# data-mermaid/mermaid-classifier

Hardware: AMD Instinct MI355X
Metric: patches/sec (224x224 EfficientNet-B0) (higher is better)
Workload: dtype f16; 1 GPU; EfficientNet-B0 forward, batch=256 random 224x224 u8 patches per GPU -> (256,1280) fp32; per_gpu_batch=256, global_batch=256, weights=synthetic seed 0, input_batches_rotated=8, lanes_per_gpu=2, parallelism=patch-sharded x1

## Files before the change

### mermaid_classifier_amd/csrc/k_mid.hip

```cpp
#include "device_common.h"

template <int CKS, int KSD, int CE>
__global__ __launch_bounds__(512) void mid14_kernel(Mid14Args a)
{
    constexpr int HW = 196, CH = 96, NCHK = CE / CH, NPF = 13, NTILE = 6 * NPF, NBAND = 5;
    constexpr int ES2 = 416;
    constexpr int R = KSD / 2, NP = KSD == 5 ? 3 : 2;
    static_assert(CE % CH == 0, "chunking");
    extern __shared__ __attribute__((aligned(16))) unsigned char smem[];
    constexpr int ZT = R, ZB = R + 1;
    unsigned char* E = smem + ZT * 7 * ES2;
    float* pband = reinterpret_cast<float*>(smem + (98 + 7 * (ZT + ZB)) * ES2);
    const int tid = threadIdx.x, lane = tid & 63, wave = __builtin_amdgcn_readfirstlane(tid >> 6);
    const int m = lane & 15, q = lane >> 4;
    const int b = blockIdx.x;
    const int Cin = a.Cin;
    const GLOBAL_AS _Float16* wexp = sgpr_ptr<_Float16>(a.wexp);
    const GLOBAL_AS float* bexp = sgpr_ptr<float>(a.bexp);
    const GLOBAL_AS uint32_t* dwp = sgpr_ptr<uint32_t>(a.dwp);
    const GLOBAL_AS float* bdw = sgpr_ptr<float>(a.bdw);
    const int npf = wave < 5 ? 2 : 1;
    const int pf0 = wave < 5 ? 2 * wave : wave + 5;
    const GLOBAL_AS _Float16* xgp = sgpr_ptr<_Float16>(a.X) + (size_t)b * HW * Cin;
    const int band0 = tid / CH, cd = tid - band0 * CH;
// ... 119 lines not shown
                        } else {
                            wq[0][0] = r0 << 16; wq[0][1] = __builtin_amdgcn_alignbit(r1, r0, 16); wq[0][2] = 0u;
                            wq[1][0] = r0; wq[1][1] = r1; wq[1][2] = 0u;
                        }
#pragma unroll
                        for (int ip = 0; ip < NP; ++ip)
#pragma unroll
                            for (int ox = 0; ox < 14; ++ox) {
                                const int fp = (KSD == 5 || !(ox & 1)) ? (ox >> 1) - 1 : (ox >> 1);
                                const int xpc = fp + ip;
                                if (xpc < 0 || xpc > 6) continue;
                                if (!started[ox]) { acc[ox] = dot2_from(P[ro + ky][xpc], wq[ox & 1][ip], dbias); started[ox] = true; }
                                else acc[ox] = __builtin_amdgcn_fdot2(*reinterpret_cast<const h2*>(&P[ro + ky][xpc]),
                                                                      *reinterpret_cast<const h2*>(&wq[ox & 1][ip]), acc[ox], false);
                            }
                    }
                    silu_scaled_staged(acc);
#pragma unroll
                    for (int ox = 0; ox < 14; ox += 2) {
                        const f2 v = {acc[ox], acc[ox + 1]};
                        psum2 = psum2 + v;
                        const uint32_t hv = cvt_pk_f16(acc[ox], acc[ox + 1]);
                        dg[(size_t)(oy * 14 + ox) * CE] = (uint16_t)hv;
                        dg[(size_t)(oy * 14 + ox + 1) * CE] = (uint16_t)(hv >> 16);
                    }
                }
            }
            pband[band * CH + cd] = (psum2.x + psum2.y) + 0.f;
        }
        T7_BAR();
        if (tid < CH)
            a.pool[(size_t)b * CE + chunk * CH + tid] =
                ((pband[tid] + pband[CH + tid]) + pband[2 * CH + tid]) + pband[3 * CH + tid] + pband[4 * CH + tid];
    }
}

template <int CKS, int KSD, int CE, bool CHAIN>
static __device__ __forceinline__ void mid14m_body(const Mid14Args& args, const int chain_tid)
{
    const Mid14Args a = args;
    constexpr bool DBG = !CHAIN;
    const int tid = CHAIN ? chain_tid : (int)threadIdx.x;
    const int by = CHAIN ? 0 : (int)blockIdx.y, ny = CHAIN ? 1 : (int)gridDim.y;
    constexpr int HW = 196, NG = CE / 16, R = KSD / 2;
    constexpr int XSTR = 64 * CKS + 16;
    constexpr int ERS = 40;
    constexpr int ECS = 736;
    constexpr int EREG = 16 * ECS;
    constexpr int TREG = 56 * 32;
    extern __shared__ __attribute__((aligned(16))) unsigned char smem[];
    unsigned char* XS = smem;
    const int lane = tid & 63, wave = __builtin_amdgcn_readfirstlane(tid >> 6);
    unsigned char* EW = smem + HW * XSTR + wave * (EREG + TREG);
    unsigned char* TW = EW + EREG;
    const int n16 = lane & 15, q = lane >> 4;
    const int blk = lane >> 2, n = lane & 3;
    const int c = 2 * (blk & 3) + ((blk >> 2) & 1) + 8 * (blk >> 3);
    const int b = blockIdx.x;
    const int Cin = a.Cin;
    const GLOBAL_AS _Float16* wexp = sgpr_ptr<_Float16>(a.wexp);
    const GLOBAL_AS float* bexp = sgpr_ptr<float>(a.bexp);
    const GLOBAL_AS _Float16* dwt = sgpr_ptr<_Float16>(a.dwdiag);
    const GLOBAL_AS float* bdw = sgpr_ptr<float>(a.bdw);
    const bool clk = DBG && a.dbg_clk != nullptr;
    long long ck[5] = {clk ? (long long)__builtin_readcyclecounter() : 0, 0, 0, 0, 0};
    {
// ... 345 lines not shown
        dbg_clk[(size_t)b * 8 + 4] = (float)((long long)__builtin_readcyclecounter() - tk0);
        dbg_clk[(size_t)b * 8 + 5] = dbg_clk[(size_t)b * 8 + 4];
    }
    static_assert(NPAIR >= 7, "waves 0..6 all own a pair of pixel fragments");
    load_chunk(wave, 0, xc);
    PIN_VMEM();
    if (k2 < KP) {
        float a0 = be0, a1 = be1;
        f4 rq[7];
#pragma unroll
        for (int j = 0; j < 7; ++j) rq[j] = *reinterpret_cast<const f4*>(rs + 4 * j);
        __builtin_amdgcn_sched_barrier(0);
#pragma unroll
        for (int j = 0; j < 28; ++j) {
            const float r = j < CSP ? rq[j >> 2][j & 3] : 0.f;
            a0 = fma_mix_lo(w2[j], r, a0);
            a1 = fma_mix_hi(w2[j], r, a1);
        }
        {
            const float g0 = fc2_thr ? sigmoid_f(a0) : 0.f, g1 = fc2_thr ? sigmoid_f(a1) : 0.f;
            gate[k2] = g0;
            gate[k2 + 1] = g1;
            if (dbg_gate && fc2_thr) {
                dbg_gate[(size_t)b * K + k2] = g0;
                dbg_gate[(size_t)b * K + k2 + 1] = g1;
            }
        }
    }
    if (dbg_clk && tid == 0) dbg_clk[(size_t)b * 8 + 6] = (float)((long long)__builtin_readcyclecounter() - tk0);
    T7_BAR();
    }
    if (dbg_clk && tid == 0) dbg_clk[(size_t)b * 8 + 7] = (float)((long long)__builtin_readcyclecounter() - tk0);
    if (dbg_clk) tk1 = (long long)__builtin_readcyclecounter();
#pragma unroll 1
    for (int pr = wave; pr < NPAIR; pr += 8) {
        f4 acc[2][NF];
#pragma unroll
        for (int i = 0; i < 2; ++i)
#pragma unroll
            for (int nf = 0; nf < NF; ++nf) acc[i][nf] = bv[nf];
        h4 rv[2][NF];
        auto load_res = [&]() {
            if (!RES) return;
            const GLOBAL_AS _Float16* rg = sgpr_ptr<_Float16>(a.res) + (size_t)b * HW * a.N;
#pragma unroll
            for (int i = 0; i < 2; ++i) {
                const int p = 32 * pr + 16 * i + m;
                const int pc = p < HW ? p : HW - 1;
#pragma unroll
                for (int nf = 0; nf < NF; ++nf) {
                    const int c = 16 * nf + 4 * q;
                    rv[i][nf] = gload<h4>(rg, (unsigned)((pc * a.N + (c < a.N ? c : 0)) * 2));
                }
            }
        };
        if (EARLY_RES) load_res();
        h8 wcur[NF];
#pragma unroll
        for (int nf = 0; nf < NF; ++nf) wcur[nf] = *reinterpret_cast<const h8*>(wl + ((nf * KS) * 64 + lane) * 16);
        f4 gc0 = *reinterpret_cast<const f4*>(gate + 8 * q), gc1 = *reinterpret_cast<const f4*>(gate + 8 * q + 4);
        long long tka = 0;
        if (dbg_clk) tka = (long long)__builtin_readcyclecounter();
#pragma unroll
        for (int ch = 0; ch < NCH; ++ch) {
            if (ch + 1 < NCH) load_chunk(pr, ch + 1, xn);
            else load_chunk(pr + 8 < NPAIR ? pr + 8 : pr, 0, xn);
#pragma unroll
            for (int u = 0; u < CK; ++u) {
                const int ks = ch * CK + u;
                const int kn = ks + 1 < KS ? ks + 1 : 0;
                h8 wnx[NF];
#pragma unroll
                for (int nf = 0; nf < NF; ++nf) wnx[nf] = *reinterpret_cast<const h8*>(wl + ((nf * KS + kn) * 64 + lane) * 16);
                const f4 gn0 = *reinterpret_cast<const f4*>(gate + 32 * kn + 8 * q);
                const f4 gn1 = *reinterpret_cast<const f4*>(gate + 32 * kn + 8 * q + 4);
                PIN_VMEM();
                h8 xb[2];
#pragma unroll
                for (int i = 0; i < 2; ++i) {
                    const uint4 o = gate_h8(*reinterpret_cast<const uint4*>(&xc[i][u]), gc0, gc1);
                    xb[i] = *reinterpret_cast<const h8*>(&o);
                }
#pragma unroll
                for (int nf = 0; nf < NF; ++nf) {
                    acc[0][nf] = __builtin_amdgcn_mfma_f32_16x16x32_f16(wcur[nf], xb[0], acc[0][nf], 0, 0, 0);
                    acc[1][nf] = __builtin_amdgcn_mfma_f32_16x16x32_f16(wcur[nf], xb[1], acc[1][nf], 0, 0, 0);
                }
                PIN_VMEM();
#pragma unroll
                for (int nf = 0; nf < NF; ++nf) wcur[nf] = wnx[nf];
                gc0 = gn0;
                gc1 = gn1;
            }
#pragma unroll
            for (int i = 0; i < 2; ++i)
#pragma unroll
                for (int u = 0; u < CK; ++u) xc[i][u] = xn[i][u];
        }
        if (dbg_clk && tid == 0) dbg_clk[(size_t)b * 8 + 2] = (float)((long long)__builtin_readcyclecounter() - tka);
        if (!EARLY_RES) load_res();
#pragma unroll
        for (int i = 0; i < 2; ++i) {
            const int p = 32 * pr + 16 * i + m;
            if (p >= HW) continue;
#pragma unroll
            for (int nf = 0; nf < NF; ++nf) {
                const int c = 16 * nf + 4 * q;
                if (c >= a.N) continue;
                float v[4];
#pragma unroll
                for (int j = 0; j < 4; ++j) v[j] = acc[i][nf][j];
                if (RES) {
#pragma unroll
                    for (int j = 0; j < 4; ++j) v[j] += (float)rv[i][nf][j];
                }
                h4 o;
#pragma unroll
                for (int j = 0; j < 4; ++j) o[j] = (_Float16)v[j];
                *reinterpret_cast<h4*>(a.Y + ((size_t)b * HW + p) * a.N + c) = o;
            }
        }
    }
    if (dbg_clk) {
        T7_BAR();
        tk2 = (long long)__builtin_readcyclecounter();
        if (tid == 0) { dbg_clk[(size_t)b * 8] = (float)(tk1 - tk0); dbg_clk[(size_t)b * 8 + 1] = (float)(tk2 - tk1); }
    }
}

template <int KS, int NF, int HW, bool RES>
__global__ __launch_bounds__(512) void proj_patch_kernel(ProjPatchArgs a)
{
    proj_patch_body<KS, NF, HW, RES, false>(a, 0);
}

enum { CH_PP_15_5_R = 0, CH_MID_3_480 = 1, CH_PP_15_7 = 2, CH_MID_4_672 = 3, CH_PP_21_7_R = 4 };
__global__ __launch_bounds__(512) void chain14_kernel(Chain14Args c)
{
#pragma unroll 1
    for (int p = 0; p < c.nph; ++p) {
        const Chain14Phase& ph = c.ph[p];
        int tid = threadIdx.x;
        asm volatile("" : "+v"(tid));
        __builtin_assume(tid >= 0 && tid < 512);
        switch (ph.kind) {
        case CH_PP_15_5_R: proj_patch_body<15, 5, 196, true, true>(ph.pp, tid); break;
        case CH_MID_3_480: mid14m_body<3, 5, 480, true>(ph.mid, tid); break;
        case CH_PP_15_7: proj_patch_body<15, 7, 196, false, true>(ph.pp, tid); break;
        case CH_MID_4_672: mid14m_body<4, 5, 672, true>(ph.mid, tid); break;
        default: proj_patch_body<21, 7, 196, true, true>(ph.pp, tid); break;
        }
        __builtin_amdgcn_sched_barrier(0);
        __syncthreads();
// ... 22 lines not shown
#define PP(KS, NF, HW, RES) {{KS, NF, HW, RES}, "proj_patch<" #KS "," #NF "," #HW "," #RES ">", launch_proj_patch_t<KS, NF, HW, RES != 0>},
static const Inst<4, ProjPatchArgs> PROJ_PATCH_TABLE[] = {
    PP(5, 3, 784, 0)
    PP(8, 3, 784, 1)
    PP(8, 5, 196, 0)
    PP(15, 5, 196, 1)
    PP(15, 7, 196, 0)
    PP(21, 7, 196, 1)
    PP(6, 4, 784, 0)
    PP(12, 4, 784, 1)
    PP(12, 7, 196, 0)
};
#undef PP

const char* proj_patch_label(int K, int N, int HW, int res) { return inst_label(PROJ_PATCH_TABLE, {proj_patch_ksteps(K), (N + 15) / 16, HW, res}); }

int launch_proj_patch(const ProjPatchArgs& a, hipStream_t st)
{
    if (a.B < 1 || a.CSP < 4 || a.CSP > 28 || (a.CSP & 3) || a.nparts < 1) return -11;
    return inst_launch(PROJ_PATCH_TABLE, {proj_patch_ksteps(a.K), (a.N + 15) / 16, a.HW, a.res ? 1 : 0}, a, st, -5);
}

template <int CKS, int KSD, int CE>
static int launch_mid14_t(const Mid14Args& a, hipStream_t st)
{
    constexpr int ZROWS = 2 * (KSD / 2) + 1;
    const int lds = (98 + 7 * ZROWS) * 416 + 5 * 96 * 4 + 512;
    if (int r = set_max_lds<&mid14_kernel<CKS, KSD, CE>>(lds)) return r;
    hipLaunchKernelGGL((mid14_kernel<CKS, KSD, CE>), dim3(a.B, a.nsplit < 1 ? 1 : a.nsplit), dim3(512), lds, st, a);
    LAUNCH_CHECK();
    return 0;
}

template <int CKS, int KSD, int CE>
static int launch_mid14m_t(const Mid14Args& a, hipStream_t st)
{
    const int lds = 196 * (64 * CKS + 16) + 8 * (16 * 736 + 56 * 32);
    if (int r = set_max_lds<&mid14m_kernel<CKS, KSD, CE>>(lds)) return r;
    hipLaunchKernelGGL((mid14m_kernel<CKS, KSD, CE>), dim3(a.B, a.nsplit < 1 ? 1 : a.nsplit), dim3(512), lds, st, a);
    LAUNCH_CHECK();
    return 0;
}

#define MID14(CKS, KSD, CE) {{CKS, KSD, CE, 0}, "mid14<" #CKS "," #KSD "," #CE ",1>", launch_mid14_t<CKS, KSD, CE>},
#define MID14M(CKS, KSD, CE) {{CKS, KSD, CE, 1}, "mid14m<" #CKS "," #KSD "," #CE ",1>", launch_mid14m_t<CKS, KSD, CE>},
static const Inst<4, Mid14Args> MID14_TABLE[] = {
    MID14(4, 5, 672) MID14M(4, 5, 672)
    MID14(3, 5, 480) MID14M(3, 5, 480)
    MID14(3, 3, 480)
};
#undef MID14M
#undef MID14

const char* mid14_label(int Cin, int ks, int Ce, int dwm) { return inst_label(MID14_TABLE, {(Cin + 31) / 32, ks, Ce, dwm}); }

int launch_mid14(const Mid14Args& a, hipStream_t st)
{
    if (a.B < 1) return -14;
    return inst_launch(MID14_TABLE, {(a.Cin + 31) / 32, a.ks, a.Ce, a.dwdiag ? 1 : 0}, a, st, -5);
}

static int proj_patch_lds(int KS, int NF) { return NF * KS * 1024 + 2 * 32 * KS * 4 + 128; }
static int mid14m_lds(int CKS) { return 196 * (64 * CKS + 16) + 8 * (16 * 736 + 56 * 32); }

int chain14_proj_kind(int K, int N, int HW, int res)
{
    const int ks = proj_patch_ksteps(K), nf = (N + 15) / 16;
    if (HW != 196) return -1;
    if (ks == 15 && nf == 5 && res) return CH_PP_15_5_R;
    if (ks == 15 && nf == 7 && !res) return CH_PP_15_7;
    if (ks == 21 && nf == 7 && res) return CH_PP_21_7_R;
    return -1;
}

int chain14_mid_kind(int Cin, int ks, int Ce)
{
    const int cks = (Cin + 31) / 32;
    if (ks != 5) return -1;
    if (cks == 3 && Ce == 480) return CH_MID_3_480;
    if (cks == 4 && Ce == 672) return CH_MID_4_672;
    return -1;
}

int launch_chain14(const Chain14Args& a, hipStream_t st)
{
    if (a.B < 1 || a.nph < 1 || a.nph > CHAIN14_MAX_PHASES) return -14;
    int lds = 0;
    for (int p = 0; p < a.nph; ++p) {
        const Chain14Phase& ph = a.ph[p];
        int need;
        if (ph.kind == CH_MID_3_480 || ph.kind == CH_MID_4_672) {
            const Mid14Args& m = ph.mid;
// ... 16 lines not shown
```

### mermaid_classifier_amd/csrc/kernels.h

```cpp
#pragma once
#include <hip/hip_runtime.h>
#include <stdint.h>

#define LAUNCH_CHECK()                          \
    do {                                        \
        hipError_t e__ = hipGetLastError();     \
        if (e__ != hipSuccess) return (int)e__; \
    } while (0)

enum { EPI_SILU = 0, EPI_LINEAR = 1, EPI_GAP = 2 };


int mmc_fail(int code, const char* fmt, ...);

struct GemmArgs {
    const _Float16* X;
    int M, K;
    const _Float16* Wp;
    int Kp;
    const float* bias;
    _Float16* Y;
    int N;
    int mt, nt, n_chunks, defer_gate;
    int epi;
// ... 104 lines not shown
    int planar;
    float* pool;
    int B;
};
int launch_mb1(const Mb1Args& a, hipStream_t st);

struct MbtArgs {
    const _Float16* X;
    const _Float16* wexp;
    const float* bexp;
    const uint32_t* dwp;
    const float* bdw;
    _Float16* D;
    float* pool;
    int B, H, Cin, Ce, ks;
    int stride;
    const _Float16* dwtoe;
};
int launch_mbt(const MbtArgs& a, hipStream_t st);
const char* mbt_label(int H, int ks, int stride, int Cin, int Ce, int dw4);

struct Mid14Args {
    const _Float16* X;
    const _Float16* wexp;
    const float* bexp;
    const uint32_t* dwp;
    const float* bdw;
    _Float16* D;
    float* pool;
    int B, Cin, Ce, ks;
    int nsplit;
    float* dbg_clk;
    const _Float16* dwdiag;
};
int launch_mid14(const Mid14Args& a, hipStream_t st);
const char* mid14_label(int Cin, int ks, int Ce, int dwm);

struct ProjPatchArgs {
    const _Float16* X;
    const float* pool_part;
    const _Float16* wr_g;
    const float* br;
    const _Float16* we_t;
    const float* be;
    const _Float16* wfrag;
    const float* bias;
    const _Float16* res;
    _Float16* Y;
    float* dbg_gate;
    float* dbg_clk;
    int B, HW, K, N, CSP, nparts;
    float psc;
};
int launch_proj_patch(const ProjPatchArgs& a, hipStream_t st);
int proj_patch_ksteps(int K);
int proj_patch_fc1_rows(int K);
const char* proj_patch_label(int K, int N, int HW, int res);

enum { CHAIN14_MAX_PHASES = 7 };
struct Chain14Phase {
    int kind;
    union {
        ProjPatchArgs pp;
        Mid14Args mid;
    };
};
struct Chain14Args {
    int B, nph;
    Chain14Phase ph[CHAIN14_MAX_PHASES];
};
int chain14_proj_kind(int K, int N, int HW, int res);
int chain14_mid_kind(int Cin, int ks, int Ce);
int launch_chain14(const Chain14Args& a, hipStream_t st);

int launch_mbconv_a(const MbArgs& a, hipStream_t st);
const char* mbconv_a_label(const MbArgs& a);
const char* mbconv_pre_label(const MbArgs& a);
const char* mbconv_d_label(const MbArgs& a);
int launch_mbconv_pre(const MbArgs& a, const _Float16* pre_w, const float* pre_b, const float* pre_gate, hipStream_t st);
int launch_mbconv_d(const MbArgs& a, hipStream_t st);
int launch_stem(const uint8_t* patches, const _Float16* w, const float* bias, const float* padval, _Float16* out, int B,
                int channels, hipStream_t st);
int launch_stem_dw(const uint8_t* patches, const _Float16* w, const float* bias, const float* padval, const float* Wdw,
                   const float* bdw, _Float16* out, float* pool_part, int B, hipStream_t st);
int launch_pw_gemm(const GemmArgs& a, hipStream_t st);
// ... 110 lines not shown
```

### mermaid_classifier_amd/csrc/mmc_api.cpp

```cpp
#include <hip/hip_runtime.h>

#include <algorithm>
#include <cmath>
#include <cstdarg>
#include <cstdio>
#include <cstdlib>
#include <cstring>
#include <map>
#include <mutex>
#include <thread>
#include <string>
#include <vector>

#include "../../include/mmc.h"
#include "api_internal.h"
#include "backbone_pack.h"
#include "kernels.h"

static const int IMG = 224;

static thread_local char g_err[512] = "";

int mmc_fail(int code, const char* fmt, ...)
{
// ... 18 lines not shown
    _Float16* w = nullptr;
    float* b = nullptr;
    const char* label[2] = {nullptr, nullptr};
};

extern "C" int mmc_fp8_e4m3_encode(const float* in, uint8_t* out, size_t n)
{
    if (!in || !out) return fail(MMC_ERR_ARG, "NULL argument");
    for (size_t i = 0; i < n; ++i) out[i] = e4m3_encode(in[i]);
    return MMC_OK;
}

static int pick_nt(int N, bool small_m)
{
    const int tiles = (N + 15) / 16;
    if (small_m) {
        int best = 4, waste = 1 << 30;
        for (int nt = 4; nt >= 2; --nt) {
            const int w = (tiles + nt - 1) / nt * nt - tiles;
            if (w < waste) { waste = w; best = nt; }
        }
        return tiles <= 4 ? tiles : best;
    }
    for (int nt = 8; nt >= 1; --nt)
        if (tiles % nt == 0) return nt;
    return 1;
}

struct Options {
    bool keep, graph, tail_clk, profile_serial;
    bool fuse, fuse_b0, mb1, mbt, mbt2, mbt4, mb_dot2, mid14, mid14m, projse, se_small, thin_proj, b1_planar;
    bool tail, tail_full, tail_b11;
    bool chain;
    int lanes, fp8_maxh;
};
static bool env_starts(const char* name, char c)
{
    const char* e = getenv(name);
    return e && e[0] == c;
}
static Options read_options()
{
    auto on = [](const char* name) { return !env_starts(name, '0'); };
    Options o;
    o.keep = env_starts("MMC_KEEP_ACTIVATIONS", '1');
    o.graph = on("MMC_GRAPH") && !o.keep;
    o.tail_clk = env_starts("MMC_TAIL_CLK", '1') && !o.keep;
    o.profile_serial = env_starts("MMC_PROFILE_SERIAL", '1');
    o.fuse = on("MMC_FUSE");
    o.fuse_b0 = on("MMC_FUSE_B0");
    o.mb1 = on("MMC_MB1");
    o.mbt = on("MMC_MBT");
    o.mbt2 = on("MMC_MBT2");
    o.mbt4 = on("MMC_MBT4");
    o.mb_dot2 = on("MMC_MB_DOT2");
    o.projse = on("MMC_PROJSE");
    o.se_small = on("MMC_SE_SMALL");
    o.thin_proj = on("MMC_THIN_PROJ");
    o.b1_planar = on("MMC_B1_PLANAR");
    o.tail = on("MMC_TAIL");
    o.tail_full = on("MMC_TAIL_FULL");
    o.tail_b11 = on("MMC_TAIL_B11");
    o.chain = on("MMC_CHAIN");
    const char* e = getenv("MMC_MID14");
    o.mid14 = !e || atoi(e) != 0;
    e = getenv("MMC_MID14M");
    o.mid14m = !e || atoi(e) >= 1;
    e = getenv("MMC_LANES");
    o.lanes = e ? atoi(e) : 2;
    e = getenv("MMC_FP8_MAXH");
    o.fp8_maxh = e && atoi(e) > 7 ? atoi(e) : 7;
    return o;
}

enum class Front {
    StemDw,
    Mbt,
    Mid14,
    Mb1,
    MbPre,
    MbD,
    MbA,
    Unfused,
    Tail,
};
enum class Back {
    ProjPatch,
    SeProject,
    SeFolded,
    Tail,
};
enum class Se { Wide, Small, Fused };
enum class Proj { Thin, Fp8, Gemm };
enum class TailRoute {
    None,
    B12,
    B11,
    B11All,
};

struct SeArgs {
    int Cs = 0;
    const float *wr = nullptr, *br = nullptr, *we = nullptr, *be = nullptr;
};

struct BlockW {
    BlockDef d;
    int H = 0, Ho = 0, ce = 0, cs = 0, cs4 = 0, pad = 0;
    bool has_expand = false, skip = false;
    int tw = 0, CG = 0, S = 0, iters = 0, parts = 0, nz = 1;
    bool fusable = false;
    bool d_fits = false;
    int d_npair = 0, d_wl_off = 0, d_red_off = 0, d_lds = 0;
    MbArgs mb{};
    Front front = Front::Unfused;
    Back back = Back::SeProject;
    Se se = Se::Fused;
    Proj proj = Proj::Gemm;
    bool mbt4 = false, mid14m = false;
    bool planar = false;
    int nparts = 0;
    const char *front_label = nullptr, *back_label = nullptr;
    PwLayer expand, project;
    float *dw_w = nullptr, *dw_b = nullptr;
    float* se_be = nullptr;
    MbtArgs mbt{};
    Mid14Args mid{};
    Mb1Args mb1{};
    DwArgs dw{};
    GemmArgs exp_gemm{};
    ProjPatchArgs pp{};
    SeArgs sea{};
    GemmArgs proj_gemm{};
    Fp8GemmArgs proj8{};
};

struct FuseCfg { int TH, TWo, CC, TW, PB; };
static const FuseCfg B0_FUSE[16] = {
    {0, 0, 0, 0, 1},     {8, 8, 48, 2, 1},    {14, 14, 48, 2, 1},  {4, 14, 48, 2, 1},   {14, 14, 48, 2, 1},
    {7, 14, 80, 2, 1},   {14, 14, 96, 2, 1},  {14, 14, 96, 2, 1},  {14, 14, 48, 2, 1},  {14, 14, 48, 2, 1},
    {14, 14, 48, 2, 1},  {7, 7, 48, 1, 1},    {7, 7, 96, 1, 2},    {7, 7, 96, 1, 2},    {7, 7, 96, 1, 2},
    {7, 7, 96, 1, 2}};
static const bool B0_DOT2[16] = {0, 0, 0, 0, 1, 0, 0, 0, 0, 1, 1, 0, 1, 1, 1, 0};

static FuseCfg generic_fuse_cfg(int H, int k, int s, int ce)
{
    FuseCfg fc{0, 0, 0, 0, 1};
    if (H == 112 && s == 2) fc = {8, 8, 48, 2, 1};
    else if (H == 56 && s == 1) fc = {14, 14, 48, 2, 1};
    else if (H == 56 && s == 2) fc = {4, 14, 48, 2, 1};
    else if (H == 28 && s == 1) fc = {14, 14, 48, 2, 1};
    else if (H == 28 && s == 2) fc = {2, 14, 48, 2, 1};
// ... 209 lines not shown
    for (int l = 0; l < 4; ++l) {
        if (bb->lanes[l].stream) hipStreamDestroy(bb->lanes[l].stream);
        if (bb->lanes[l].done) hipEventDestroy(bb->lanes[l].done);
    }
    if (bb->fork) hipEventDestroy(bb->fork);
    if (bb->last_done) hipEventDestroy(bb->last_done);
    for (auto& g : bb->graphs) hipGraphExecDestroy(g.exec);
    if (bb->gstream) hipStreamDestroy(bb->gstream);
    delete bb;
}

extern "C" int mmc_backbone_create(const void* packed, size_t nbytes, int arch, int device, int max_batch,
                                   mmc_backbone** out)
{
    return mmc_backbone_create_ex(packed, nbytes, arch, device, max_batch, 0u, out);
}

static int gemm_defer_gate(bool gate, int HW) { return (gate && HW <= 49) ? 1 : 0; }

static bool plan_gemm(PwLayer& L, int epi, bool gate, bool res, int HW)
{
    L.label[0] = pw_gemm_label(1, L.nt, epi, gate, res, gemm_defer_gate(gate, HW));
    L.label[1] = epi == EPI_GAP ? L.label[0] : pw_gemm_label(2, L.nt, epi, gate, res, 0);
    return L.label[0] && L.label[1] && (epi != EPI_GAP || HW <= 64);
}

static int plan_block(const mmc_backbone* bb, BlockW& B, int i)
{
    const Options& o = bb->opt;
    const bool is_b0 = bb->arch == MMC_ARCH_B0;
    const int HWo = B.Ho * B.Ho;
    const bool tail_blk = (bb->tail == TailRoute::B11All && i >= 11) || (bb->tail != TailRoute::None && i >= 12);
    const bool mbt = o.fuse && o.mbt && (B.d.s == 1 || o.mbt2) && mbt_label(B.H, B.d.k, B.d.s, B.d.cin, B.ce, 0);
    const bool mid14 = is_b0 && o.fuse && o.projse && o.mid14 && i >= 6 && i <= 10 && mid14_label(B.d.cin, B.d.k, B.ce, 0);
    if (i == 0 && bb->fuse_stem) B.front = Front::StemDw;
    else if (tail_blk) B.front = Front::Tail;
    else if (B.fusable && mbt) B.front = Front::Mbt;
    else if (B.fusable && mid14) B.front = Front::Mid14;
    else if (B.fusable && is_b0 && o.mb_dot2 && B0_DOT2[i] && B.d_fits) B.front = Front::MbD;
    else if (B.fusable && i == 1 && bb->fuse_b0b1) B.front = o.mb1 ? Front::Mb1 : Front::MbPre;
    else if (B.fusable) B.front = Front::MbA;
    else B.front = Front::Unfused;
    B.mbt4 = B.front == Front::Mbt && o.mbt4 && B.ce % 16 == 0 && mbt_label(B.H, B.d.k, B.d.s, B.d.cin, B.ce, 1);
    B.mid14m = B.front == Front::Mid14 && o.mid14m && i >= 8 && B.ce % 16 == 0 && mid14_label(B.d.cin, B.d.k, B.ce, 1);
    if (B.front == Front::MbD) {
        B.mb.npair = B.d_npair; B.mb.wl_off = B.d_wl_off; B.mb.red_off = B.d_red_off; B.mb.lds_bytes = B.d_lds;
    }
    const char* family = nullptr;
    const int tiles = B.mb.tiles_x * B.mb.tiles_y;
    switch (B.front) {
    case Front::StemDw: B.nparts = 49; break;
    case Front::Mb1: B.nparts = 14; break;
    case Front::Tail: B.nparts = B.parts; break;
    case Front::Mbt:
        B.nparts = B.d.s == 2 ? (B.Ho / 7) * (B.Ho / 14) : (B.H / 14) * (B.H / 28);
        B.front_label = mbt_label(B.H, B.d.k, B.d.s, B.d.cin, B.ce, B.mbt4);
        break;
    case Front::Mid14: B.nparts = 1; B.front_label = mid14_label(B.d.cin, B.d.k, B.ce, B.mid14m); break;
    case Front::MbPre: B.nparts = tiles; family = "mbconv_a PRE"; B.front_label = mbconv_pre_label(B.mb); break;
    case Front::MbD: B.nparts = tiles; family = "mbconv_d"; B.front_label = mbconv_d_label(B.mb); break;
    case Front::MbA: B.nparts = tiles; family = "mbconv_a"; B.front_label = mbconv_a_label(B.mb); break;
    case Front::Unfused:
        B.nparts = B.parts;
        family = "dwconv";
        B.front_label = dwconv_label(B.d.k, B.d.s, B.tw);
        if (B.front_label && B.has_expand && !plan_gemm(B.expand, EPI_SILU, false, false, B.H * B.H)) {
            family = "pw_gemm (expand)";
            B.front_label = nullptr;
        }
        break;
    }
    if (family && !B.front_label)
        return fail(MMC_ERR_ARG, "block %d: no %s instantiation for %dx%d, kernel %d, stride %d, %d -> %d channels (tile %dx%d, chunk %d)",
                    i, family, B.H, B.H, B.d.k, B.d.s, B.d.cin, B.ce, B.mb.TH, B.mb.TWo, B.mb.CC);
    const bool fp8_blk = bb->fp8 && B.Ho <= o.fp8_maxh;
    const char* pp = proj_patch_label(B.ce, B.d.cout, HWo, B.skip ? 1 : 0);
    const bool proj_patch = o.fuse && o.projse && B.fusable && B.has_expand && B.cs4 <= 28 && pp && (is_b0 ? i >= 3 && i <= 10 : !fp8_blk);
    if (tail_blk || (i == 11 && bb->tail == TailRoute::B11)) B.back = Back::Tail;
    else if (proj_patch) B.back = Back::ProjPatch;
    else if (i == 0 && bb->fuse_b0b1) B.back = Back::SeFolded;
    else B.back = Back::SeProject;
    B.back_label = B.back == Back::ProjPatch ? pp : nullptr;
    B.se = !is_b0 ? Se::Wide : (o.se_small && B.ce <= 256 && B.cs <= 16) ? Se::Small : Se::Fused;
    PwLayer& P = B.project;
    const bool thin = o.thin_proj && P.nt == 2 && P.n_chunks == 1 && thin_proj_label(P.Kp / 32, B.skip ? 1 : 0) && P.N <= 32 &&
                      (P.N & 7) == 0 && (HWo & 15) == 0 && HWo >= 3136;
    B.proj = thin ? Proj::Thin : fp8_blk ? Proj::Fp8 : Proj::Gemm;
    if (B.back == Back::SeProject && B.proj == Proj::Gemm && !plan_gemm(P, EPI_LINEAR, true, B.skip, HWo))
        return fail(MMC_ERR_ARG, "block %d: no pw_gemm (project) instantiation for %d -> %d channels at %dx%d", i, B.ce, B.d.cout, B.Ho, B.Ho);
    B.planar = B.front == Front::Mb1 && thin && o.b1_planar && !o.keep && P.K == 96;
    return 0;
// ... 33 lines not shown
    BIND(dev_upload(bb, we_t, pack_se_fc2_t16(R.se_we, B.ce, B.cs, B.cs4)));
    return dev_upload(bb, br, pack_bias(R.se_br, B.cs, B.cs4 > 32 ? B.cs4 : 32, 1.0));
}

static int bind_shared(mmc_backbone* bb, BlockW& B, int i, const RawBlock& R)
{
    if (B.has_expand) BIND(upload_pw(bb, &B.expand, pack_pw(R.exp_w, R.exp_b, B.ce, B.d.cin, B.expand.nt, LOG2E, LOG2E)));
    BIND(dev_upload(bb, &B.dw_w, pack_dw_taps(R.dw_w, B.ce, B.d.k, dw_tap_scale(B, i))));
    BIND(dev_upload(bb, &B.dw_b, pack_bias(R.dw_b, B.ce, B.ce, LOG2E)));
    BIND(dev_upload(bb, &B.se_be, pack_bias(R.se_be, B.ce, B.ce, 1.0)));
    return upload_pw(bb, &B.project, pack_pw(R.proj_w, R.proj_b, B.d.cout, B.ce, B.project.nt, 1.0 / LOG2E, 1.0));
}

static int bind_mbt(mmc_backbone* bb, BlockW& B, int i, const RawBlock& R)
{
    MbtArgs& a = B.mbt;
    BIND(upload_exp_frag(bb, B, R, &a.wexp));
    BIND(dev_upload(bb, &a.dwp, pack_dw_pairs(R.dw_w, B.ce, B.d.k)));
    if (B.mbt4) BIND(dev_upload(bb, &a.dwtoe, pack_dw_toeplitz(R.dw_w, B.ce, B.d.k, dw_tap_scale(B, i))));
    a.bexp = B.expand.b; a.bdw = B.dw_b;
    a.H = B.H; a.Cin = B.d.cin; a.Ce = B.ce; a.ks = B.d.k; a.stride = B.d.s;
    return 0;
}

static int bind_mid14(mmc_backbone* bb, BlockW& B, int i, const RawBlock& R)
{
    Mid14Args& a = B.mid;
    BIND(upload_exp_frag(bb, B, R, &a.wexp));
    BIND(upload_dw_requests(bb, B, R, &a.dwp));
    if (B.mid14m) BIND(dev_upload(bb, &a.dwdiag, pack_dw_toeplitz(R.dw_w, B.ce, B.d.k, dw_tap_scale(B, i))));
    a.bexp = B.expand.b; a.bdw = B.dw_b;
    a.Cin = B.d.cin; a.Ce = B.ce; a.ks = B.d.k;
    a.nsplit = B.mid14m ? 1 : 4;
    return 0;
}

static int bind_mb1(mmc_backbone* bb, BlockW& B, const RawNet& raw)
{
    const int kp = 32 * B.mb.ksteps;
    Mb1Args& m = B.mb1;
    BIND(dev_upload(bb, &m.pre_w, pack_frag(raw.blk[0].proj_w, 16, 32, 32, 1, 1, 1.0 / LOG2E)));
    const std::vector<_Float16> wn = pack_expand_rows(raw.blk[1].exp_w, B.ce, B.d.cin, kp);
    BIND(dev_upload(bb, &m.wexp, pack_expand_kperm(wn.data(), B.ce, kp)));
    m.pre_b = bb->blk[0].project.b; m.bexp = B.expand.b; m.wdw = B.dw_w; m.bdw = B.dw_b;
    m.planar = B.planar ? 1 : 0;
    if (B.front == Front::MbPre) {
        MbArgs& a = B.mb;
        a.Cin = 32; a.Wexp = m.wexp; a.bexp = B.expand.b; a.Wdw = B.dw_w; a.bdw = B.dw_b;
    }
    return 0;
}

static int bind_mb(mmc_backbone* bb, BlockW& B, const RawBlock& R)
{
    MbArgs& a = B.mb;
    BIND(dev_upload(bb, &a.Wexp, pack_expand_rows(R.exp_w, B.ce, B.d.cin, 32 * a.ksteps)));
    a.bexp = B.expand.b; a.Wdw = B.dw_w; a.bdw = B.dw_b;
    return 0;
}

static int bind_unfused(BlockW& B)
{
    if (B.has_expand) B.exp_gemm = gemm_args(B.expand, EPI_SILU, false, B.H * B.H);
    DwArgs& d = B.dw;
    d.wt = B.dw_w; d.bias = B.dw_b;
    d.H = B.H; d.W = B.H; d.C = B.ce; d.Ho = B.Ho; d.Wo = B.Ho; d.pad_t = B.pad; d.pad_l = B.pad;
// ... 15 lines not shown
    BIND(upload_dw_requests(bb, B, R, &t.dwp));
    t.bexp = B.expand.b; t.bdw = B.dw_b; t.ks = B.d.k;
    return 0;
}

static int bind_front(mmc_backbone* bb, BlockW& B, int i, const RawNet& raw)
{
    const RawBlock& R = raw.blk[i];
    switch (B.front) {
    case Front::StemDw: return 0;
    case Front::Mbt: return bind_mbt(bb, B, i, R);
    case Front::Mid14: return bind_mid14(bb, B, i, R);
    case Front::Mb1: case Front::MbPre: return bind_mb1(bb, B, raw);
    case Front::MbD: case Front::MbA: return bind_mb(bb, B, R);
    case Front::Unfused: return bind_unfused(B);
    case Front::Tail: return bind_tail_front(bb, B, i, R);
    }
    return 0;
}

static int bind_proj_patch(mmc_backbone* bb, BlockW& B, const RawBlock& R)
{
    ProjPatchArgs& a = B.pp;
    const _Float16* wr_t = nullptr;
    BIND(upload_se_t16(bb, B, R, &wr_t, &a.we_t, &a.br));
    const std::vector<_Float16> wrt = pack_se_fc1_t16(R.se_wr, B.ce, B.cs, B.cs4);
    BIND(dev_upload(bb, &a.wr_g, pack_se_fc1_groups(wrt.data(), B.ce, B.cs4, proj_patch_fc1_rows(B.ce))));
    const int nf = (B.d.cout + 15) / 16;
    BIND(dev_upload(bb, &a.wfrag, pack_frag(R.proj_w, B.d.cout, B.ce, B.ce, nf, proj_patch_ksteps(B.ce), 1.0 / LOG2E)));
    BIND(dev_upload(bb, &a.bias, pack_bias(R.proj_b, B.d.cout, 16 * nf, 1.0)));
    a.be = B.se_be;
    a.HW = B.Ho * B.Ho; a.K = B.ce; a.N = B.d.cout; a.CSP = B.cs4; a.nparts = B.nparts;
    a.psc = (float)(1.0 / ((double)a.HW * LOG2E));
    return 0;
}

static int bind_se(mmc_backbone* bb, BlockW& B, const RawBlock& R)
{
    SeArgs& s = B.sea;
    const double psc = 1.0 / ((double)B.Ho * B.Ho * LOG2E);
    s.be = B.se_be;
    switch (B.se) {
    case Se::Fused:
        BIND(dev_upload(bb, &s.wr, pack_se_fc1_frag(R.se_wr, B.ce, B.cs, psc)));
        BIND(dev_upload(bb, &s.we, pack_se_fc2_frag(R.se_we, B.ce, B.cs)));
        BIND(dev_upload(bb, &s.br, pack_bias(R.se_br, B.cs, B.cs > 48 ? B.cs : 48, 1.0)));
        s.Cs = B.cs4;
        return 0;
    case Se::Small:
        BIND(dev_upload(bb, &s.wr, pack_se_fc1_nat(R.se_wr, B.ce, B.cs, psc)));
        BIND(dev_upload(bb, &s.we, std::vector<float>(R.se_we, R.se_we + (size_t)B.ce * B.cs)));
        break;
    case Se::Wide:
        BIND(dev_upload(bb, &s.wr, pack_se_fc1_nat(R.se_wr, B.ce, B.cs, psc)));
        BIND(dev_upload(bb, &s.we, pack_se_fc2_t(R.se_we, B.ce, B.cs)));
        break;
    }
    s.Cs = B.cs;
    return dev_upload(bb, &s.br, pack_bias(R.se_br, B.cs, B.cs, 1.0));
}

static int bind_project(mmc_backbone* bb, BlockW& B, const RawBlock& R)
{
    const int HWo = B.Ho * B.Ho;
    switch (B.proj) {
    case Proj::Thin: case Proj::Gemm: B.proj_gemm = gemm_args(B.project, EPI_LINEAR, true, HWo); return 0;
// ... 144 lines not shown
                add(bn(i, ".mbconv"), B.front_label, Op::Mid14).a.mid = a;
            break;
        }
        case Front::Mb1: {
            Mb1Args& a = add("b0.project+b1.mbconv", "mb1", Op::Mb1).a.mb1 = B.mb1;
            a.X = y; a.pre_gate = ws.gate; a.D = D; a.pool = pool;
            break;
        }
        case Front::MbPre: {
            MbPreArgs& a = add("b0.project+b1.mbconv", B.front_label, Op::MbPre).a.pre = {B.mb, B.mb1.pre_w, B.mb1.pre_b, ws.gate};
            a.mb.X = y; a.mb.out = D; a.mb.pool_part = pool;
            break;
        }
        case Front::MbD: case Front::MbA: {
            MbArgs& a = add(bn(i, ".mbconv"), B.front_label, B.front == Front::MbD ? Op::MbD : Op::MbA).a.mb = B.mb;
            a.X = x; a.out = D; a.pool_part = pool;
            break;
        }
        case Front::Unfused: {
            const _Float16* dw_in = x;
            if (B.has_expand) {
                GemmArgs& g = add_gemm(bn(i, ".expand"), B.expand, B.exp_gemm, HWi);
                g.X = x; g.Y = ws.expbuf;
                writes(ws.expbuf, (size_t)HWi * B.ce, bn(i, ".expand"));
                dw_in = ws.expbuf;
            }
            DwArgs& d = add(bn(i, ".dw"), B.front_label, Op::Dw).a.dw = B.dw;
            d.in = dw_in; d.out = D; d.pool_part = pool;
            break;
        }
        case Front::Tail: break;
        }
        writes(D, (size_t)HWo * B.ce, bn(i, ".dw"));
        writes(pool, (size_t)B.nparts * B.ce);
        if (B.back == Back::Tail) break;
        if (B.back == Back::ProjPatch) {
            ProjPatchArgs pa = B.pp;
            pa.X = D; pa.pool_part = pool; pa.res = B.skip ? x : nullptr; pa.Y = y;
            pa.dbg_gate = bb->keep ? ws.gate : nullptr;
            pa.dbg_clk = bb->keep ? bb->dbg_clk : nullptr;
            if (chained) {
                if (i == ch0) {
                    xbase = x; ybase = y;
                    add(bn(ch0, ".projse-") + bn(ch1, ".projse.chain"), "chain14", Op::Chain14);
                }
                pa.Y = ch_act(ybase, B.d.cout);
                Chain14Args& ca = list.back().a.chain;
                ca.ph[ca.nph].kind = chain14_proj_kind(pa.K, pa.N, pa.HW, pa.res ? 1 : 0);
                ca.ph[ca.nph++].pp = pa;
                writes(pa.Y, (size_t)HWo * B.d.cout);
                x = pa.Y;
                std::swap(xbase, ybase);
                y = ybase;
                continue;
            }
            add(bn(i, ".projse"), B.back_label, Op::ProjPatch).a.pp = pa;
            writes(ws.gate, (size_t)B.ce, bn(i, ".gate"));
            writes(y, (size_t)HWo * B.d.cout, bn(i, ".out"));
            if (bb->keep) list.back().keep.push_back({bn(i, ".clk"), bb->dbg_clk, 8, false});
            std::swap(x, y);
            continue;
        }
        add(bn(i, ".gate"), B.se == Se::Wide ? "se_wide" : B.se == Se::Small ? "se_small" : "se_fused",
            B.se == Se::Wide ? Op::SeWide : B.se == Se::Small ? Op::SeSmall : Op::SeFused).a.se = {pool, B.nparts, B.ce, B.sea, ws.gate};
        writes(ws.gate, (size_t)B.ce, bn(i, ".gate"));
        if (B.back == Back::SeFolded) continue;
        const _Float16* res = B.skip ? x : nullptr;
// ... 708 lines not shown
```

Measured before the change: 237,900 patches/s.

## Add even-split mid14 kernel and split the odd last pixel pair in proj_patch

Adds a mid14e kernel for the 3x3 stride-1 480-channel mid-block. It splits channels into 48-wide units across a second grid dimension, hands each wave an equal share of expand tiles, and splits the depthwise work into two column halves so all 8 waves stay busy. In proj_patch, the trailing odd pixel pair (13 fragments) is no longer run by one wave; it is spread across up to 4 waves, one per output fragment, to shrink the tail imbalance. Both paths are on by default through MMC_EVEN_SPLIT. The cost is more blocks that each recompute weight loads, plus some redundant input loads.

```diff
diff --git a/mermaid_classifier_amd/csrc/k_mid.hip b/mermaid_classifier_amd/csrc/k_mid.hip
--- a/mermaid_classifier_amd/csrc/k_mid.hip
+++ b/mermaid_classifier_amd/csrc/k_mid.hip
@@ -175,6 +175,165 @@
         if (tid < CH)
             a.pool[(size_t)b * CE + chunk * CH + tid] =
                 ((pband[tid] + pband[CH + tid]) + pband[2 * CH + tid]) + pband[3 * CH + tid] + pband[4 * CH + tid];
+    }
+}
+
+template <int CKS, int CE>
+__global__ __launch_bounds__(512) void mid14e_kernel(Mid14Args a)
+{
+    constexpr int HW = 196, CH = 48, NWF = CH / 16, NPF = 13, NTILE = NWF * NPF, TPW = 5, NBAND = 5;
+    constexpr int ES2 = 224;
+    static_assert(CE % CH == 0, "units");
+    static_assert(8 * TPW >= NTILE && 7 * TPW < NTILE, "every wave owns at least one tile");
+    extern __shared__ __attribute__((aligned(16))) unsigned char smem[];
+    constexpr int ZT = 1, ZB = 2;
+    unsigned char* E = smem + ZT * 7 * ES2;
+    float* pband = reinterpret_cast<float*>(smem + (98 + 7 * (ZT + ZB)) * ES2);
+    const int tid = threadIdx.x, lane = tid & 63, wave = __builtin_amdgcn_readfirstlane(tid >> 6);
+    const int m = lane & 15, q = lane >> 4;
+    const int b = blockIdx.x, unit = blockIdx.y;
+    const int Cin = a.Cin;
+    const GLOBAL_AS _Float16* wexp = sgpr_ptr<_Float16>(a.wexp);
+    const GLOBAL_AS float* bexp = sgpr_ptr<float>(a.bexp);
+    const GLOBAL_AS uint32_t* dwp = sgpr_ptr<uint32_t>(a.dwp);
+    const GLOBAL_AS float* bdw = sgpr_ptr<float>(a.bdw);
+    const GLOBAL_AS _Float16* xgp = sgpr_ptr<_Float16>(a.X) + (size_t)b * HW * Cin;
+    const int idx = tid & 255;
+    const int band0 = idx / CH, cd = idx - band0 * CH;
+    const int band = band0 < NBAND ? band0 : NBAND - 1;
+    const int rb = 3 * band;
+    for (int e = tid; e < (ZT + ZB) * 7 * (ES2 / 16); e += 512) {
+        const int row = e / (ES2 / 16), c16 = e - row * (ES2 / 16);
+        unsigned char* zr = smem + (row < ZT * 7 ? row : row + 98) * ES2 + 16 * c16;
+        *reinterpret_cast<uint4*>(zr) = uint4{0u, 0u, 0u, 0u};
+    }
+    uint32_t raw[9];
+    const int cg = unit * CH + cd;
+#pragma unroll
+    for (int i = 0; i < 9; ++i) raw[i] = gload<uint32_t>(dwp, (unsigned)(((i >> 2) * CE + cg) * 4 + (i & 3)) * 4u);
+    const float dbias = gload<float>(bdw, (unsigned)cg * 4u);
+    {
+        const int t0 = TPW * wave;
+        const int nfa = t0 / NPF;
+        unsigned char* const scratch = reinterpret_cast<unsigned char*>(pband + 2 * NBAND * CH) + lane * 4;
+        auto expand_unit = [&](auto sw_tag) {
+            constexpr int SW = decltype(sw_tag)::value;
+            constexpr int NW = SW < TPW ? 2 : 1;
+            h8 w[NW][CKS];
+            float bs[NW];
+#pragma unroll
+            for (int j = 0; j < NW; ++j) {
+                const int nfg = NWF * unit + nfa + j;
+                bs[j] = gload<float>(bexp, (unsigned)(16 * nfg + m) * 4u);
+#pragma unroll
+                for (int ks = 0; ks < CKS; ++ks) w[j][ks] = gload<h8>(wexp, (unsigned)(((nfg * CKS + ks) * 64 + lane) * 16));
+            }
+            h8 xb[TPW][CKS];
+            int pf[TPW];
+#pragma unroll
+            for (int i = 0; i < TPW; ++i) {
+                const int t = t0 + i < NTILE ? t0 + i : NTILE - 1;
+                pf[i] = t - NPF * (nfa + (i >= SW ? 1 : 0));
+                const int pix = 16 * pf[i] + m;
+                const int pixc = pix < HW ? pix : HW - 1;
+#pragma unroll
+                for (int ks = 0; ks < CKS; ++ks) {
+                    const int kk = 32 * ks + 8 * q;
+                    xb[i][ks] = gload<h8>(xgp, (unsigned)((pixc * Cin + (kk < Cin ? kk : Cin - 8)) * 2));
+                }
+            }
+            PIN_VMEM();
+            float t[4 * TPW];
+#pragma unroll
+            for (int i = 0; i < TPW; ++i) {
+                const int j = i >= SW ? 1 : 0;
+                const f4 bv = {bs[j], bs[j], bs[j], bs[j]};
+                f4 acc = __builtin_amdgcn_mfma_f32_16x16x32_f16(xb[i][0], w[j][0], bv, 0, 0, 0);
+#pragma unroll
+                for (int ks = 1; ks < CKS; ++ks) acc = __builtin_amdgcn_mfma_f32_16x16x32_f16(xb[i][ks], w[j][ks], acc, 0, 0, 0);
+#pragma unroll
+                for (int e = 0; e < 4; ++e) t[4 * i + e] = acc[e];
+            }
+            silu_scaled_staged(t);
+#pragma unroll
+            for (int i = 0; i < TPW; ++i) {
+                const int nf = nfa + (i >= SW ? 1 : 0);
+                const int pix0 = 16 * pf[i] + 4 * q;
+                const h2 p0 = {(_Float16)t[4 * i], (_Float16)t[4 * i + 1]};
+                const h2 p1 = {(_Float16)t[4 * i + 2], (_Float16)t[4 * i + 3]};
+                const bool ok = pix0 < HW;
+                unsigned char* dst = E + (pix0 >> 1) * ES2 + (16 * nf + m) * 4;
+                *reinterpret_cast<h2*>(ok ? dst : scratch) = p0;
+                *reinterpret_cast<h2*>(ok ? dst + ES2 : scratch + 256) = p1;
+            }
+        };
+        static_assert(NPF == 13 && TPW == 5, "which waves straddle");
+        if (wave == 2) expand_unit(std::integral_constant<int, 3>{});
+        else if (wave == 5) expand_unit(std::integral_constant<int, 1>{});
+        else expand_unit(std::integral_constant<int, TPW>{});
+    }
+    T7_BAR();
+    auto depthwise = [&](auto half_tag) {
+        constexpr int HALF = decltype(half_tag)::value;
+        constexpr int X0 = 7 * HALF;
+        constexpr int PL = HALF ? 3 : 0;
+        const unsigned char* col = E + 4 * cd + ((rb - 1) * 7 + PL) * ES2;
+        uint32_t P[5][4];
+#pragma unroll
+        for (int r = 0; r < 5; ++r)
+#pragma unroll
+            for (int pp = 0; pp < 4; ++pp) P[r][pp] = *reinterpret_cast<const uint32_t*>(col + (r * 7 + pp) * ES2);
+        f2 psum2 = {0.f, 0.f};
+        float psum1 = 0.f;
+        uint16_t* dg = reinterpret_cast<uint16_t*>(a.D + (size_t)b * HW * CE + unit * CH + cd);
+#pragma unroll
+        for (int ro = 0; ro < 3; ++ro) {
+            const int oy = rb + ro;
+            if (oy < 14) {
+                float acc[7];
+                bool started[7] = {false, false, false, false, false, false, false};
+#pragma unroll
+                for (int ky = 0; ky < 3; ++ky) {
+                    const uint32_t r0 = raw[3 * ky], r1 = raw[3 * ky + 1];
+                    uint32_t wq[2][2];
+                    wq[0][0] = r0 << 16; wq[0][1] = __builtin_amdgcn_alignbit(r1, r0, 16);
+                    wq[1][0] = r0; wq[1][1] = r1;
+#pragma unroll
+                    for (int ip = 0; ip < 2; ++ip)
+#pragma unroll
+                        for (int l = 0; l < 7; ++l) {
+                            const int ox = X0 + l;
+                            const int fp = !(ox & 1) ? (ox >> 1) - 1 : (ox >> 1);
+                            const int xpc = fp + ip;
+                            if (xpc < 0 || xpc > 6) continue;
+                            if (!started[l]) { acc[l] = dot2_from(P[ro + ky][xpc - PL], wq[ox & 1][ip], dbias); started[l] = true; }
+                            else acc[l] = __builtin_amdgcn_fdot2(*reinterpret_cast<const h2*>(&P[ro + ky][xpc - PL]),
+                                                                 *reinterpret_cast<const h2*>(&wq[ox & 1][ip]), acc[l], false);
+                        }
+                }
+                silu_scaled_staged(acc);
+#pragma unroll
+                for (int l = 0; l < 6; l += 2) {
+                    const f2 v = {acc[l], acc[l + 1]};
+                    psum2 = psum2 + v;
+                    const uint32_t hv = cvt_pk_f16(acc[l], acc[l + 1]);
+                    dg[(size_t)(oy * 14 + X0 + l) * CE] = (uint16_t)hv;
+                    dg[(size_t)(oy * 14 + X0 + l + 1) * CE] = (uint16_t)(hv >> 16);
+                }
+                psum1 += acc[6];
+                dg[(size_t)(oy * 14 + X0 + 6) * CE] = (uint16_t)cvt_pk_f16(acc[6], acc[6]);
+            }
+        }
+        pband[(2 * band + HALF) * CH + cd] = ((psum2.x + psum2.y) + psum1) + 0.f;
+    };
+    if (wave < 4) depthwise(std::integral_constant<int, 0>{});
+    else depthwise(std::integral_constant<int, 1>{});
+    T7_BAR();
+    if (tid < CH) {
+        float s = pband[tid];
+#pragma unroll
+        for (int j = 1; j < 2 * NBAND; ++j) s += pband[j * CH + tid];
+        a.pool[(size_t)b * CE + unit * CH + tid] = s;
     }
 }
 
@@ -586,8 +745,10 @@
     }
     if (dbg_clk && tid == 0) dbg_clk[(size_t)b * 8 + 7] = (float)((long long)__builtin_readcyclecounter() - tk0);
     if (dbg_clk) tk1 = (long long)__builtin_readcyclecounter();
+    constexpr bool SPLIT_LAST = !CHAIN && (NPF & 1) && NPAIR > 8;
+    const int npm = SPLIT_LAST && a.even ? NPAIR - 1 : NPAIR;
 #pragma unroll 1
-    for (int pr = wave; pr < NPAIR; pr += 8) {
+    for (int pr = wave; pr < npm; pr += 8) {
         f4 acc[2][NF];
 #pragma unroll
         for (int i = 0; i < 2; ++i)
@@ -618,7 +779,7 @@
 #pragma unroll
         for (int ch = 0; ch < NCH; ++ch) {
             if (ch + 1 < NCH) load_chunk(pr, ch + 1, xn);
-            else load_chunk(pr + 8 < NPAIR ? pr + 8 : pr, 0, xn);
+            else load_chunk(pr + 8 < npm ? pr + 8 : (SPLIT_LAST && npm < NPAIR ? NPAIR - 1 : pr), 0, xn);
 #pragma unroll
             for (int u = 0; u < CK; ++u) {
                 const int ks = ch * CK + u;
@@ -673,6 +834,54 @@
                 for (int j = 0; j < 4; ++j) o[j] = (_Float16)v[j];
                 *reinterpret_cast<h4*>(a.Y + ((size_t)b * HW + p) * a.N + c) = o;
             }
+        }
+    }
+    if constexpr (SPLIT_LAST) {
+        static_assert(NF <= 4, "one wave per output fragment of the last pixel fragment");
+        auto last_fragment = [&](auto nfo_tag) {
+            constexpr int NFO = decltype(nfo_tag)::value;
+            const int p = 16 * (NPF - 1) + m;
+            const int c = 16 * NFO + 4 * q;
+            h4 rv;
+            if (RES) {
+                const GLOBAL_AS _Float16* rg = sgpr_ptr<_Float16>(a.res) + (size_t)b * HW * a.N;
+                rv = gload<h4>(rg, (unsigned)(((p < HW ? p : HW - 1) * a.N + (c < a.N ? c : 0)) * 2));
+            }
+            f4 acc = bv[NFO];
+#pragma unroll
+            for (int ch = 0; ch < NCH; ++ch) {
+                if (ch + 1 < NCH) load_chunk(NPAIR - 1, ch + 1, xn);
+#pragma unroll
+                for (int u = 0; u < CK; ++u) {
+                    const int ks = ch * CK + u;
+                    const h8 w = *reinterpret_cast<const h8*>(wl + ((NFO * KS + ks) * 64 + lane) * 16);
+                    const f4 g0 = *reinterpret_cast<const f4*>(gate + 32 * ks + 8 * q);
+                    const f4 g1 = *reinterpret_cast<const f4*>(gate + 32 * ks + 8 * q + 4);
+                    const uint4 o = gate_h8(*reinterpret_cast<const uint4*>(&xc[0][u]), g0, g1);
+                    acc = __builtin_amdgcn_mfma_f32_16x16x32_f16(w, *reinterpret_cast<const h8*>(&o), acc, 0, 0, 0);
+                }
+#pragma unroll
+                for (int u = 0; u < CK; ++u) xc[0][u] = xn[0][u];
+            }
+            if (p < HW && c < a.N) {
+                float v[4];
+#pragma unroll
+                for (int j = 0; j < 4; ++j) v[j] = acc[j];
+                if (RES) {
+#pragma unroll
+                    for (int j = 0; j < 4; ++j) v[j] += (float)rv[j];
+                }
+                h4 o;
+#pragma unroll
+                for (int j = 0; j < 4; ++j) o[j] = (_Float16)v[j];
+                *reinterpret_cast<h4*>(a.Y + ((size_t)b * HW + p) * a.N + c) = o;
+            }
+        };
+        if (npm < NPAIR) {
+            if (wave == 0) last_fragment(std::integral_constant<int, 0>{});
+            if constexpr (NF > 1) { if (wave == 1) last_fragment(std::integral_constant<int, 1>{}); }
+            if constexpr (NF > 2) { if (wave == 2) last_fragment(std::integral_constant<int, 2>{}); }
+            if constexpr (NF > 3) { if (wave == 3) last_fragment(std::integral_constant<int, 3>{}); }
         }
     }
     if (dbg_clk) {
@@ -761,6 +970,16 @@
     return 0;
 }
 
+template <int CKS, int CE>
+static int launch_mid14e_t(const Mid14Args& a, hipStream_t st)
+{
+    const int lds = (98 + 7 * 3) * 224 + 10 * 48 * 4 + 512;
+    if (int r = set_max_lds<&mid14e_kernel<CKS, CE>>(lds)) return r;
+    hipLaunchKernelGGL((mid14e_kernel<CKS, CE>), dim3(a.B, CE / 48), dim3(512), lds, st, a);
+    LAUNCH_CHECK();
+    return 0;
+}
+
 template <int CKS, int KSD, int CE>
 static int launch_mid14m_t(const Mid14Args& a, hipStream_t st)
 {
@@ -771,22 +990,24 @@
     return 0;
 }
 
-#define MID14(CKS, KSD, CE) {{CKS, KSD, CE, 0}, "mid14<" #CKS "," #KSD "," #CE ",1>", launch_mid14_t<CKS, KSD, CE>},
-#define MID14M(CKS, KSD, CE) {{CKS, KSD, CE, 1}, "mid14m<" #CKS "," #KSD "," #CE ",1>", launch_mid14m_t<CKS, KSD, CE>},
+#define MID14(CKS, KSD, CE) {{CKS, KSD, CE, MID14_PLAIN}, "mid14<" #CKS "," #KSD "," #CE ",1>", launch_mid14_t<CKS, KSD, CE>},
+#define MID14M(CKS, KSD, CE) {{CKS, KSD, CE, MID14_DWM}, "mid14m<" #CKS "," #KSD "," #CE ",1>", launch_mid14m_t<CKS, KSD, CE>},
+#define MID14E(CKS, CE) {{CKS, 3, CE, MID14_EVEN}, "mid14e<" #CKS ",3," #CE ",1>", launch_mid14e_t<CKS, CE>},
 static const Inst<4, Mid14Args> MID14_TABLE[] = {
     MID14(4, 5, 672) MID14M(4, 5, 672)
     MID14(3, 5, 480) MID14M(3, 5, 480)
-    MID14(3, 3, 480)
+    MID14(3, 3, 480) MID14E(3, 480)
 };
+#undef MID14E
 #undef MID14M
 #undef MID14
 
-const char* mid14_label(int Cin, int ks, int Ce, int dwm) { return inst_label(MID14_TABLE, {(Cin + 31) / 32, ks, Ce, dwm}); }
+const char* mid14_label(int Cin, int ks, int Ce, int form) { return inst_label(MID14_TABLE, {(Cin + 31) / 32, ks, Ce, form}); }
 
 int launch_mid14(const Mid14Args& a, hipStream_t st)
 {
     if (a.B < 1) return -14;
-    return inst_launch(MID14_TABLE, {(a.Cin + 31) / 32, a.ks, a.Ce, a.dwdiag ? 1 : 0}, a, st, -5);
+    return inst_launch(MID14_TABLE, {(a.Cin + 31) / 32, a.ks, a.Ce, a.dwdiag ? MID14_DWM : a.even ? MID14_EVEN : MID14_PLAIN}, a, st, -5);
 }
 
 static int proj_patch_lds(int KS, int NF) { return NF * KS * 1024 + 2 * 32 * KS * 4 + 128; }
diff --git a/mermaid_classifier_amd/csrc/kernels.h b/mermaid_classifier_amd/csrc/kernels.h
--- a/mermaid_classifier_amd/csrc/kernels.h
+++ b/mermaid_classifier_amd/csrc/kernels.h
@@ -160,9 +160,11 @@
     int nsplit;
     float* dbg_clk;
     const _Float16* dwdiag;
-};
+    int even;
+};
+enum { MID14_PLAIN = 0, MID14_DWM = 1, MID14_EVEN = 2 };
 int launch_mid14(const Mid14Args& a, hipStream_t st);
-const char* mid14_label(int Cin, int ks, int Ce, int dwm);
+const char* mid14_label(int Cin, int ks, int Ce, int form);
 
 struct ProjPatchArgs {
     const _Float16* X;
@@ -179,6 +181,7 @@
     float* dbg_clk;
     int B, HW, K, N, CSP, nparts;
     float psc;
+    int even;
 };
 int launch_proj_patch(const ProjPatchArgs& a, hipStream_t st);
 int proj_patch_ksteps(int K);
diff --git a/mermaid_classifier_amd/csrc/mmc_api.cpp b/mermaid_classifier_amd/csrc/mmc_api.cpp
--- a/mermaid_classifier_amd/csrc/mmc_api.cpp
+++ b/mermaid_classifier_amd/csrc/mmc_api.cpp
@@ -74,8 +74,10 @@
     bool fuse, fuse_b0, mb1, mbt, mbt2, mbt4, mb_dot2, mid14, mid14m, projse, se_small, thin_proj, b1_planar;
     bool tail, tail_full, tail_b11;
     bool chain;
+    int even_split;
     int lanes, fp8_maxh;
 };
+enum { EVEN_PROJ = 2, EVEN_B6 = 4, EVEN_B7 = 8, EVEN_ALL = EVEN_PROJ | EVEN_B6 | EVEN_B7 };
 static bool env_starts(const char* name, char c)
 {
     const char* e = getenv(name);
@@ -104,7 +106,9 @@
     o.tail_full = on("MMC_TAIL_FULL");
     o.tail_b11 = on("MMC_TAIL_B11");
     o.chain = on("MMC_CHAIN");
-    const char* e = getenv("MMC_MID14");
+    const char* e = getenv("MMC_EVEN_SPLIT");
+    o.even_split = !e || atoi(e) == 1 ? EVEN_ALL : atoi(e) & EVEN_ALL;
+    e = getenv("MMC_MID14");
     o.mid14 = !e || atoi(e) != 0;
     e = getenv("MMC_MID14M");
     o.mid14m = !e || atoi(e) >= 1;
@@ -160,6 +164,7 @@
     Se se = Se::Fused;
     Proj proj = Proj::Gemm;
     bool mbt4 = false, mid14m = false;
+    bool mid14e = false;
     bool planar = false;
     int nparts = 0;
     const char *front_label = nullptr, *back_label = nullptr;
@@ -435,7 +440,7 @@
     const int HWo = B.Ho * B.Ho;
     const bool tail_blk = (bb->tail == TailRoute::B11All && i >= 11) || (bb->tail != TailRoute::None && i >= 12);
     const bool mbt = o.fuse && o.mbt && (B.d.s == 1 || o.mbt2) && mbt_label(B.H, B.d.k, B.d.s, B.d.cin, B.ce, 0);
-    const bool mid14 = is_b0 && o.fuse && o.projse && o.mid14 && i >= 6 && i <= 10 && mid14_label(B.d.cin, B.d.k, B.ce, 0);
+    const bool mid14 = is_b0 && o.fuse && o.projse && o.mid14 && i >= 6 && i <= 10 && mid14_label(B.d.cin, B.d.k, B.ce, MID14_PLAIN);
     if (i == 0 && bb->fuse_stem) B.front = Front::StemDw;
     else if (tail_blk) B.front = Front::Tail;
     else if (B.fusable && mbt) B.front = Front::Mbt;
@@ -445,7 +450,7 @@
     else if (B.fusable) B.front = Front::MbA;
     else B.front = Front::Unfused;
     B.mbt4 = B.front == Front::Mbt && o.mbt4 && B.ce % 16 == 0 && mbt_label(B.H, B.d.k, B.d.s, B.d.cin, B.ce, 1);
-    B.mid14m = B.front == Front::Mid14 && o.mid14m && i >= 8 && B.ce % 16 == 0 && mid14_label(B.d.cin, B.d.k, B.ce, 1);
+    B.mid14m = B.front == Front::Mid14 && o.mid14m && i >= 8 && B.ce % 16 == 0 && mid14_label(B.d.cin, B.d.k, B.ce, MID14_DWM);
     if (B.front == Front::MbD) {
         B.mb.npair = B.d_npair; B.mb.wl_off = B.d_wl_off; B.mb.red_off = B.d_red_off; B.mb.lds_bytes = B.d_lds;
     }
@@ -459,7 +464,11 @@
         B.nparts = B.d.s == 2 ? (B.Ho / 7) * (B.Ho / 14) : (B.H / 14) * (B.H / 28);
         B.front_label = mbt_label(B.H, B.d.k, B.d.s, B.d.cin, B.ce, B.mbt4);
         break;
-    case Front::Mid14: B.nparts = 1; B.front_label = mid14_label(B.d.cin, B.d.k, B.ce, B.mid14m); break;
+    case Front::Mid14:
+        B.mid14e = !B.mid14m && (o.even_split & (i == 6 ? EVEN_B6 : EVEN_B7)) && mid14_label(B.d.cin, B.d.k, B.ce, MID14_EVEN);
+        B.nparts = 1;
+        B.front_label = mid14_label(B.d.cin, B.d.k, B.ce, B.mid14m ? MID14_DWM : B.mid14e ? MID14_EVEN : MID14_PLAIN);
+        break;
     case Front::MbPre: B.nparts = tiles; family = "mbconv_a PRE"; B.front_label = mbconv_pre_label(B.mb); break;
     case Front::MbD: B.nparts = tiles; family = "mbconv_d"; B.front_label = mbconv_d_label(B.mb); break;
     case Front::MbA: B.nparts = tiles; family = "mbconv_a"; B.front_label = mbconv_a_label(B.mb); break;
@@ -559,6 +568,7 @@
     a.bexp = B.expand.b; a.bdw = B.dw_b;
     a.Cin = B.d.cin; a.Ce = B.ce; a.ks = B.d.k;
     a.nsplit = B.mid14m ? 1 : 4;
+    a.even = B.mid14e ? 1 : 0;
     return 0;
 }
 
@@ -640,6 +650,7 @@
     a.be = B.se_be;
     a.HW = B.Ho * B.Ho; a.K = B.ce; a.N = B.d.cout; a.CSP = B.cs4; a.nparts = B.nparts;
     a.psc = (float)(1.0 / ((double)a.HW * LOG2E));
+    a.even = (bb->opt.even_split & EVEN_PROJ) ? 1 : 0;
     return 0;
 }
 
@@ -850,7 +861,7 @@
         case Front::Tail: break;
         }
         writes(D, (size_t)HWo * B.ce, bn(i, ".dw"));
-        writes(pool, (size_t)B.nparts * B.ce);
+        writes(pool, (size_t)B.nparts * B.ce, B.front == Front::Mid14 ? bn(i, ".pool") : std::string());
         if (B.back == Back::Tail) break;
         if (B.back == Back::ProjPatch) {
             ProjPatchArgs pa = B.pp;
```

Result: slower. 227,200 patches/s (-4.5%).
